# PeixinC/VoiceControlledRobot-VAR

Hardware: AMD Instinct MI355X
Metric: pretext triplets/sec (84x84 RGB + 16 kHz/1 s audio) (higher is better)
Workload: dtype f32; 1 GPU; Kuka+GoogleCommand pretext step, batch 256 per GPU on MI355X, fp32: u8 84x84 image + 2 int16 1 s clips per triplet resident in HBM -> MFCC -> fwd + triplet loss + bwd + Adam (BASELINE.json configs[1]); per_gpu_batch=256, global_batch=256, audio=16 kHz x 1 s int16 x 2, parallelism=dp1, launch=hip-graph replay, head=triplet

## Files before the change

### voicecontrolledrobot-var_amd/csrc/img_tail2.hip

```cpp
#include <stdlib.h>

#include <type_traits>

#include "var_common.h"

namespace {
PH_DECL();
}
#ifdef VAR_PHASES
extern "C" int var_debug_phases_tail2(unsigned long long* out) {
    unsigned long long z[32] = {0};
    if (hipMemcpyFromSymbol(out, HIP_SYMBOL(g_phase), sizeof(z)) != hipSuccess) return -1;
    return hipMemcpyToSymbol(HIP_SYMBOL(g_phase), z, sizeof(z)) == hipSuccess ? 0 : -1;
}
#endif
namespace {
typedef float f32x4t __attribute__((ext_vector_type(4)));

template <bool U8_, int H1_, int RB_, bool TILED_>
struct Tail2Cfg {
    static constexpr bool U8 = U8_, TILED = TILED_;
    static constexpr int CH = 32, H1 = H1_, W1 = H1_, HI = 2 * H1_, HO2 = H1_ / 2;
    static constexpr int RB = RB_, R2 = RB_ / 2, NB = H1_ / RB_;
    static constexpr int A1_ROWS = RB + 1, A1_PITCH = W1, A1_ROW0 = (W1 % 4 == 2) ? 2 : 4;
    static constexpr int A1_PLANE = TILED ? ((A1_ROW0 + A1_ROWS * W1 + 7) / 8) * 8 + 4 : A1_ROW0 + A1_ROWS * W1;
    static constexpr int A1_FLOATS = CH * A1_PLANE;
    static constexpr int G2_ROWS = R2 + 1, G2_PITCH = HO2 + 1;
    static constexpr int G2_PLANE = ((G2_ROWS * G2_PITCH + 15) / 32) * 32 + 16, G2_FLOATS = CH * G2_PLANE;
    static constexpr int G1_PLANE = RB * W1 + ((RB * W1) % 32 == 0 ? 4 : 0), G1_FLOATS = CH * G1_PLANE;
    static constexpr int IM_ROWS = 2 * RB + 1, IM_PITCH = HI + 4, IM_PLANE = IM_ROWS * IM_PITCH, IM_FLOATS = 3 * IM_PLANE;
    static constexpr bool PIPE = !TILED_;
    static constexpr int NBUF = PIPE ? 2 : 1;
    static constexpr int A1S = 0, G2S = A1S + 2 * A1_FLOATS, G1S = G2S + 2 * G2_FLOATS, IMS = G1S + NBUF * G1_FLOATS;
    static constexpr int LUT = IMS + NBUF * IM_FLOATS, ZCELL = LUT + 256;
    static constexpr int LDS_FLOATS = ZCELL + 4;
    static constexpr int LDS_BYTES = LDS_FLOATS * 4;
    static constexpr int NPX2 = R2 * HO2;
    static constexpr int NT2 = (NPX2 + 15) / 16;
    static constexpr int TPW = NT2 % 2 == 0 ? 2 : 1;
    static constexpr int NACC = TPW == 1 ? 2 : 1;
    static constexpr int ND = 2 * NT2 / TPW;
    static constexpr int NT = 64 * (ND + 8);
    static constexpr int KS_W = (NPX2 + 3) / 4;
    static constexpr int NPX1 = RB * W1;
    static constexpr int KS_1 = NPX1 / 4;
    static constexpr int SK = KS_1 <= 48 ? KS_1 / 4 : 8;
    static constexpr int DK = KS_1 <= 48 ? 0 : (((KS_1 - 32 + ND - 1) / ND + 3) / 4) * 4;
    static constexpr int NSL = 4 + (DK ? ND : 0);
    static constexpr int N_A1 = A1_FLOATS / 4;
    static constexpr int P4 = A1_PLANE / 4;
    static constexpr int N_G2 = CH * G2_ROWS * HO2;
    static constexpr int N_IM = 3 * IM_ROWS * (HI / 4);
    static constexpr int L_A1 = TILED ? (N_A1 + 255) / 256 : CH / 4;
    static constexpr int L_G2 = (N_G2 + 255) / 256, L_IM = (N_IM + 255) / 256;
    static constexpr int SLAB0 = 32 * 32 + 32, SLAB1 = 32 * 9 * 32 + 32;
    static_assert(H1 % RB == 0 && RB % 2 == 0 && NPX1 % 4 == 0 && A1_PLANE % 4 == 0 && 4 * SK + DK * ND >= KS_1 && (SK == 8 || SK == 12) && (DK == 0 || DK == 8), "bands, k-step shares");
    static_assert(NT <= 1024 && LDS_BYTES <= 160 * 1024, "one workgroup per CU");
    static_assert(PIPE == (DK == 0), "the pipelined form is the one where role S holds all of conv 1's weight gradient");
    static_assert(NSL * 1024 + NSL * 32 <= 2 * A1_FLOATS, "the end-of-kernel fold scratch aliases the act1 buffers");
    static_assert(CH * HO2 * HO2 < (1 << 15) && CH * G2_PLANE < (1 << 12) && G2_ROWS <= 4, "role S: packed gact2 element table");
    static_assert(3 * HI * HI < (1 << 15) && 3 * IM_PLANE < (1 << 12) && IM_ROWS <= 16, "role S: packed image group table");
};

template <class C>
__global__ void __launch_bounds__(C::NT)
img_tail2_kernel(const float* __restrict__ gy, const float* __restrict__ wd, const float* __restrict__ act1,
                 const void* __restrict__ image, long bstride, const int* __restrict__ bidx,
                 float* __restrict__ slabs0, float* __restrict__ slabs1, int B) {
    extern __shared__ __attribute__((aligned(16))) float lds[];
    using XT = typename std::conditional<C::U8, uint8_t, float>::type;
    const int tid = threadIdx.x, lane = tid & 63, wave = tid >> 6;
    const int q = lane >> 4, l15 = lane & 15;
    const float* lut = lds + C::LUT;
    const int nimg = ((int)blockIdx.x < B) ? (B - 1 - (int)blockIdx.x) / (int)gridDim.x + 1 : 0;
    const int ntl = nimg * C::NB;
    auto tile_img = [&](int j) { return (int)blockIdx.x + (j / C::NB) * (int)gridDim.x; };

    PHR_INIT(3, VAR_PH_THREAD);
    if (tid < 256) lds[C::LUT + tid] = (float)tid / 255.f;
    if (tid < 4) lds[C::ZCELL + tid] = 0.f;
    for (int e = tid; e < 2 * C::G2_FLOATS; e += C::NT) lds[C::G2S + e] = 0.f;
    for (int e = tid; e < C::NBUF * 3 * C::IM_ROWS; e += C::NT) lds[C::IMS + e * C::IM_PITCH + 3] = 0.f;
    __syncthreads();

    float* slab0 = slabs0 + (size_t)blockIdx.x * C::SLAB0;
    float* slab1 = slabs1 + (size_t)blockIdx.x * C::SLAB1;
    f32x4t s_acc[2][2];
    float s_bs[2] = {0.f, 0.f};
#pragma unroll
    for (int a = 0; a < 2; ++a)
#pragma unroll
        for (int b = 0; b < 2; ++b) s_acc[a][b] = {0.f, 0.f, 0.f, 0.f};

    int cbase[2];
#pragma unroll
    for (int kt = 0; kt < 2; ++kt) {
        int col = 16 * kt + l15;
        col = col > 26 ? 26 : col;
        const int tap = col / 3, c = col - tap * 3;
        cbase[kt] = C::IMS + c * C::IM_PLANE + (tap / 3) * C::IM_PITCH + (tap % 3) + 3;
    }
    auto wgrad1_chunk = [&](auto ck, int s_lo, int s_hi, int opq, int g1o = 0, int imo = 0) {
        int m = 4 * s_lo + q + opq;
        int yl = m / C::W1, x = m - yl * C::W1;
        const int ga = C::G1S + g1o + l15 * C::G1_PLANE;
        constexpr int CK = decltype(ck)::value;
        float a0[CK], a1v[CK], b0[CK], b1[CK];
#pragma unroll
        for (int u = 0; u < CK; ++u) {
            const bool live = s_lo + u < s_hi;
            const int pix = 2 * yl * C::IM_PITCH + 2 * x;
            const int ao = live ? ga + m : C::ZCELL, po = live ? pix : 0;
            a0[u] = lds[ao];
            a1v[u] = lds[live ? ao + 16 * C::G1_PLANE : C::ZCELL];
            b0[u] = lds[cbase[0] + imo + po];
            b1[u] = lds[cbase[1] + imo + po];
            m += 4; x += 4;
            if (x >= C::W1) { x -= C::W1; ++yl; }
        }
        __builtin_amdgcn_sched_barrier(0);
#pragma unroll
        for (int u = 0; u < CK; ++u) {
            s_bs[0] += a0[u]; s_bs[1] += a1v[u];
            s_acc[0][0] = __builtin_amdgcn_mfma_f32_16x16x4f32(a0[u], b0[u], s_acc[0][0], 0, 0, 0);
            s_acc[0][1] = __builtin_amdgcn_mfma_f32_16x16x4f32(a0[u], b1[u], s_acc[0][1], 0, 0, 0);
            s_acc[1][0] = __builtin_amdgcn_mfma_f32_16x16x4f32(a1v[u], b0[u], s_acc[1][0], 0, 0, 0);
            s_acc[1][1] = __builtin_amdgcn_mfma_f32_16x16x4f32(a1v[u], b1[u], s_acc[1][1], 0, 0, 0);
        }
        __builtin_amdgcn_sched_barrier(0);
    };

    auto g2_load = [&](auto nl, float* r, int j, int lt) {
        constexpr int NL = decltype(nl)::value, WIN = C::G2_ROWS * C::HO2, CPP = NL / WIN, L = (C::CH + CPP - 1) / CPP;
        const int band = j % C::NB, b = tile_img(j);
        const int cs = lt / WIN, w = lt - cs * WIN, rr = w / C::HO2;
        const int back = (C::R2 * band + rr >= C::HO2) ? C::HO2 : 0;
        const float* pg = gy + (size_t)b * C::CH * C::HO2 * C::HO2 + C::R2 * band * C::HO2 + cs * C::HO2 * C::HO2 + w - back;
#pragma unroll
        for (int i = 0; i < L; ++i) {
            const bool ok = cs < CPP && cs + CPP * i < C::CH;
            r[i] = pg[ok ? CPP * i * C::HO2 * C::HO2 : 0];
        }
    };
    auto g2_store = [&](auto nl, const float* r, int j, int lt) {
        constexpr int NL = decltype(nl)::value, WIN = C::G2_ROWS * C::HO2, CPP = NL / WIN, L = (C::CH + CPP - 1) / CPP;
        const int band = j % C::NB;
        const int cs = lt / WIN, w = lt - cs * WIN, rr = w / C::HO2, ox = w - rr * C::HO2;
        float* dg = lds + C::G2S + (j & 1) * C::G2_FLOATS + cs * C::G2_PLANE + rr * C::G2_PITCH + ox;
        const bool live = C::R2 * band + rr < C::HO2;
#pragma unroll
        for (int i = 0; i < L; ++i)
            if (cs < CPP && cs + CPP * i < C::CH) dg[CPP * i * C::G2_PLANE] = live ? r[i] : 0.f;
    };
    constexpr bool G2_IN_D = C::DK == 0;
    constexpr int NLD_ = 64 * C::ND, L_G2D = (C::CH + NLD_ / (C::G2_ROWS * C::HO2) - 1) / (NLD_ / (C::G2_ROWS * C::HO2));

    auto park_slices = [&](int sl) {
        float* d = lds + sl * 1024;
#pragma unroll
        for (int a = 0; a < 2; ++a)
#pragma unroll
            for (int b = 0; b < 2; ++b)
#pragma unroll
                for (int r = 0; r < 4; ++r) d[(16 * a + 4 * q + r) * 32 + 16 * b + l15] = s_acc[a][b][r];
        float b0 = s_bs[0], b1 = s_bs[1];
        b0 += __shfl_xor(b0, 16, 64); b0 += __shfl_xor(b0, 32, 64);
        b1 += __shfl_xor(b1, 16, 64); b1 += __shfl_xor(b1, 32, 64);
        if (q == 0) { lds[C::NSL * 1024 + sl * 32 + l15] = b0; lds[C::NSL * 1024 + sl * 32 + 16 + l15] = b1; }
    };

    if (wave < C::ND) {
        const int ct = wave & 1, pp = wave >> 1;
        float A[72];
#pragma unroll
        for (int t = 0; t < 72; ++t) A[t] = wd[((t >> 3) * 32 + 4 * (t & 7) + q) * 32 + 16 * ct + l15];
#pragma unroll
        for (int t = 0; t < 72; ++t) asm volatile("" : "+v"(A[t]));
        int mj[C::TPW], mi[C::TPW];
        bool mok[C::TPW];
#pragma unroll
        for (int u = 0; u < C::TPW; ++u) {
            int m = (C::TPW * pp + u) * 16 + l15;
            mok[u] = m < C::NPX2;
            if (!mok[u]) m = 0;
            mj[u] = m / C::HO2; mi[u] = m - mj[u] * C::HO2;
        }
        __syncthreads();
        PHR(0);
        for (int j = 0; j < ntl; ++j) {
            __syncthreads();
            PHR(1);
            float r_g2d[G2_IN_D ? L_G2D : 1];
            int dtid = tid;
            if constexpr (G2_IN_D) {
                asm volatile("" : "+v"(dtid));
                if (j + 1 < ntl) g2_load(std::integral_constant<int, NLD_>{}, r_g2d, j + 1, dtid);
            }
            const int g2 = C::G2S + (j & 1) * C::G2_FLOATS + q * C::G2_PLANE;
            const int a1 = C::A1S + (j & 1) * C::A1_FLOATS;
            constexpr int kCls[9] = {0, 1, 1, 2, 2, 3, 3, 3, 3};
            constexpr int kKy[9] = {1, 1, 1, 0, 2, 0, 0, 2, 2}, kKx[9] = {1, 0, 2, 1, 1, 0, 2, 0, 2};
            int mjb[C::TPW], mib[C::TPW], lb[C::TPW];
#pragma unroll
            for (int u = 0; u < C::TPW; ++u) {
                mjb[u] = mj[u]; mib[u] = mi[u];
                asm volatile("" : "+v"(mjb[u])); asm volatile("" : "+v"(mib[u]));
                lb[u] = g2 + mjb[u] * C::G2_PITCH + mib[u];
            }
            float bb[2][C::TPW][4];
            auto fetch = [&](int buf, int h) {
                const int k = h >> 1, s0 = 4 * (h & 1);
                const int off = (kKy[k] == 0 ? C::G2_PITCH : 0) + (kKx[k] == 0 ? 1 : 0);
#pragma unroll
                for (int ss = 0; ss < 4; ++ss) {
                    bb[buf][0][ss] = lds[lb[0] + off + 4 * (s0 + ss) * C::G2_PLANE];
                    if constexpr (C::TPW == 2) bb[buf][C::TPW - 1][ss] = lds[lb[C::TPW - 1] + off + 4 * (s0 + ss) * C::G2_PLANE];
                }
            };
            f32x4t acc[C::TPW * C::NACC];
#pragma unroll
            for (int u = 0; u < C::TPW * C::NACC; ++u) acc[u] = {0.f, 0.f, 0.f, 0.f};
            fetch(0, 0);
#pragma unroll
            for (int h = 0; h < 18; ++h) {
                const int k = h >> 1;
                if (h + 1 < 18) fetch((h + 1) & 1, h + 1);
                __builtin_amdgcn_sched_barrier(0);
                const int tap = kKy[k] * 3 + kKx[k];
#pragma unroll
                for (int ss = 0; ss < 4; ++ss)
#pragma unroll
                    for (int u = 0; u < C::TPW; ++u)
                        acc[u * C::NACC + ss % C::NACC] = __builtin_amdgcn_mfma_f32_16x16x4f32(A[tap * 8 + 4 * (h & 1) + ss], bb[h & 1][u][ss],
                                                                                    acc[u * C::NACC + ss % C::NACC], 0, 0, 0);
                __builtin_amdgcn_sched_barrier(0);
                if (!(h & 1)) continue;
                if (k + 1 == 9 || kCls[k + 1] != kCls[k]) {
                    const int py = kCls[k] >> 1, px = kCls[k] & 1;
#pragma unroll
                    for (int u = 0; u < C::TPW; ++u) {
                        f32x4t tot = acc[u * C::NACC];
                        if constexpr (C::NACC == 2) tot += acc[u * C::NACC + 1];
                        const int yl = 2 * mjb[u] + py, x = 2 * mib[u] + px;
                        const int mo = a1 + (16 * ct + 4 * q) * C::A1_PLANE + C::A1_ROW0 + (yl + 1) * C::A1_PITCH + x;
                        const int go = C::G1S + (C::PIPE ? (j & 1) * C::G1_FLOATS : 0) + (16 * ct + 4 * q) * C::G1_PLANE + yl * C::W1 + x;
                        float mv[4];
#pragma unroll
                        for (int r = 0; r < 4; ++r) mv[r] = lds[mo + r * C::A1_PLANE];
                        if (mok[u]) {
#pragma unroll
                            for (int r = 0; r < 4; ++r) lds[go + r * C::G1_PLANE] = mv[r] > 0.f ? tot[r] : 0.f;
                        }
#pragma unroll
                        for (int a = 0; a < C::NACC; ++a) acc[u * C::NACC + a] = {0.f, 0.f, 0.f, 0.f};
                    }
                }
            }
            if constexpr (G2_IN_D) {
                asm volatile("" : "+v"(dtid));
                if (j + 1 < ntl) g2_store(std::integral_constant<int, NLD_>{}, r_g2d, j + 1, dtid);
            }
            PHR(2);
            if constexpr (!C::PIPE) __syncthreads();
            PHR(3);
            if constexpr (C::DK == 8) {
                wgrad1_chunk(std::integral_constant<int, 4>{}, 32 + 8 * wave, 32 + 8 * wave + 4, 0);
                wgrad1_chunk(std::integral_constant<int, 4>{}, 32 + 8 * wave + 4, 32 + 8 * wave + 8 < C::KS_1 ? 32 + 8 * wave + 8 : C::KS_1, 0);
            }
            PHR(4);
        }
        PHR_FLUSH();
        if constexpr (C::PIPE) __syncthreads();
        if constexpr (C::DK == 0) __syncthreads();
    } else if (wave < C::ND + 4) {
        const int w = wave - C::ND, nt = w & 1, ctl = w >> 1;
        int aoff[C::KS_W], boff[C::KS_W];
        uint32_t edge = 0;
#pragma unroll
        for (int s = 0; s < C::KS_W; ++s) {
            const int m = 4 * s + q;
            const bool ok = m < C::NPX2;
            const int mm = ok ? m : 0;
            const int r = mm / C::HO2, ox = mm - r * C::HO2;
            aoff[s] = ok ? (16 * nt + l15) * C::G2_PLANE + r * C::G2_PITCH + ox : -1;
            boff[s] = (16 * ctl + l15) * C::A1_PLANE + C::A1_ROW0 + 2 * r * C::A1_PITCH + 2 * ox - 1;
            if (ox == 0) edge |= 1u << s;
        }
        f32x4t acc[9];
#pragma unroll
        for (int t = 0; t < 9; ++t) acc[t] = {0.f, 0.f, 0.f, 0.f};
        float bsum = 0.f;
        __syncthreads();
        PHR(0);
        for (int j = 0; j < ntl; ++j) {
            __syncthreads();
            PHR(1);
            const int g2 = C::G2S + (j & 1) * C::G2_FLOATS, a1 = C::A1S + (j & 1) * C::A1_FLOATS;
            float av[2], bv[2][9];
            auto fetch = [&](int buf, int ss) {
                av[buf] = lds[aoff[ss] < 0 ? C::ZCELL : g2 + aoff[ss]];
#pragma unroll
                for (int t = 0; t < 9; ++t) {
                    const float v = lds[a1 + boff[ss] + (t / 3) * C::A1_PITCH + (t % 3)];
                    bv[buf][t] = (t % 3 == 0 && ((edge >> ss) & 1)) ? 0.f : v;
                }
            };
            fetch(0, 0);
#pragma unroll
            for (int ss = 0; ss < C::KS_W; ++ss) {
                if (ss + 1 < C::KS_W) fetch((ss + 1) & 1, ss + 1);
                __builtin_amdgcn_sched_barrier(0);
                bsum += av[ss & 1];
#pragma unroll
                for (int t = 0; t < 9; ++t) acc[t] = __builtin_amdgcn_mfma_f32_16x16x4f32(av[ss & 1], bv[ss & 1][t], acc[t], 0, 0, 0);
                __builtin_amdgcn_sched_barrier(0);
                if (ss + 1 == C::KS_W / 2) { PHR(2); if constexpr (!C::PIPE) __syncthreads(); PHR(3); }
            }
            PHR(4);
        }
#pragma unroll
        for (int t = 0; t < 9; ++t)
#pragma unroll
            for (int r = 0; r < 4; ++r) slab1[((16 * nt + 4 * q + r) * 9 + t) * 32 + 16 * ctl + l15] = acc[t][r];
        bsum += __shfl_xor(bsum, 16, 64);
        bsum += __shfl_xor(bsum, 32, 64);
        if (ctl == 0 && q == 0) slab1[9216 + 16 * nt + l15] = bsum;
        PHR_FLUSH();
        if constexpr (C::PIPE) __syncthreads();
        if constexpr (C::DK == 0) __syncthreads();
    } else {
        const int sw = wave - C::ND - 4, stid0 = tid - 64 * (C::ND + 4);
        float r_g2[C::L_G2];
        uint32_t r_u8[C::U8 ? C::L_IM : 1];
        float4 r_f4[C::U8 ? 1 : C::L_IM];
        auto make_g2 = [&](int e) -> uint32_t {
            const int ee = e < C::N_G2 ? e : 0;
            const int ch = ee / (C::G2_ROWS * C::HO2), rem = ee - ch * (C::G2_ROWS * C::HO2);
            const int r = rem / C::HO2, ox = rem - r * C::HO2;
            return (uint32_t)(ch * C::HO2 * C::HO2 + r * C::HO2 + ox) | ((uint32_t)(ch * C::G2_PLANE + r * C::G2_PITCH + ox) << 15) |
                   ((uint32_t)r << 27) | (e < C::N_G2 ? 0u : 0x80000000u);
        };
        auto make_im = [&](int e) -> uint32_t {
            const int ee = e < C::N_IM ? e : 0;
            const int c = ee / (C::IM_ROWS * (C::HI / 4)), rem = ee - c * (C::IM_ROWS * (C::HI / 4));
            const int r = rem / (C::HI / 4), g = rem - r * (C::HI / 4);
            return (uint32_t)(c * C::HI * C::HI + r * C::HI + 4 * g) | ((uint32_t)(c * C::IM_PLANE + r * C::IM_PITCH + 4 + 4 * g) << 15) |
                   ((uint32_t)r << 27) | (e < C::N_IM ? 0u : 0x80000000u);
        };
        constexpr bool TAB = C::DK != 0;
        uint32_t t_g2[TAB ? C::L_G2 : 1], t_im[TAB ? C::L_IM : 1];
        if constexpr (TAB) {
#pragma unroll
            for (int i = 0; i < C::L_G2; ++i) t_g2[i] = make_g2(stid0 + 256 * i);
#pragma unroll
            for (int i = 0; i < C::L_IM; ++i) t_im[i] = make_im(stid0 + 256 * i);
        }
        auto e_g2 = [&](int i, int stid) -> uint32_t { if constexpr (TAB) return t_g2[i]; else return make_g2(stid + 256 * i); };
        static_assert(TAB || (C::L_IM == 3 && C::IM_ROWS * (C::HI / 4) <= 256), "image band: a channel per pass");
        auto e_im = [&](int i, int stid) -> uint32_t {
            if constexpr (TAB) return t_im[i];
            else return stid < C::IM_ROWS * (C::HI / 4) ? make_im(stid) : 0x80000000u;
        };
        auto issue_a1g2 = [&](int j, int stid, bool with_g2 = true) {
            const int band = j % C::NB, b = tile_img(j);
            const float* pa = C::TILED ? act1 + (size_t)b * kAct1TiledFloats + (size_t)band * C::A1_FLOATS
                                       : act1 + (size_t)b * C::CH * C::H1 * C::W1;
            float* da = lds + C::A1S + (j & 1) * C::A1_FLOATS;
#pragma unroll
            for (int i = 0; i < C::L_A1; ++i) {
                const int k = sw + 4 * i;
                if constexpr (C::TILED) {
                    if (k * 64 + lane < C::N_A1)
                        __builtin_amdgcn_global_load_lds((const __attribute__((address_space(1))) void*)(pa + k * 256 + 4 * lane),
                                                         (__attribute__((address_space(3))) void*)(da + k * 256), 16, 0, 0);
                } else {
                    static_assert(C::TILED || (C::P4 <= 64 && C::L_A1 * 4 == C::CH), "NCHW gather: a channel per instruction");
                    int off = k * C::H1 * C::W1 + (C::RB * band - 1) * C::W1 - C::A1_ROW0 + 4 * lane;
                    off = off < 0 ? 0 : off;
                    if (lane < C::P4)
                        __builtin_amdgcn_global_load_lds((const __attribute__((address_space(1))) void*)(pa + off),
                                                         (__attribute__((address_space(3))) void*)(da + k * C::A1_PLANE), 16, 0, 0);
                }
            }
            if (!with_g2) return;
            const float* pg = gy + (size_t)b * C::CH * C::HO2 * C::HO2 + C::R2 * band * C::HO2;
#pragma unroll
            for (int i = 0; i < C::L_G2; ++i) {
                const uint32_t tg = e_g2(i, stid);
                const int r = (tg >> 27) & 3;
                const int back = (C::R2 * band + r >= C::HO2) ? C::HO2 : 0;
                r_g2[i] = pg[(int)(tg & 0x7fff) - back];
            }
        };
        auto store_a1g2 = [&](int j, int stid) {
            const int band = j % C::NB;
            float* dg = lds + C::G2S + (j & 1) * C::G2_FLOATS;
#pragma unroll
            for (int i = 0; i < C::L_G2; ++i) {
                const uint32_t tg = e_g2(i, stid);
                const int r = (tg >> 27) & 3;
                if (!(tg >> 31)) dg[(tg >> 15) & 0xfff] = (C::R2 * band + r < C::HO2) ? r_g2[i] : 0.f;
            }
        };
        auto issue_img = [&](int j, int stid) {
            const int band = j % C::NB, b = tile_img(j);
            const int gi = bidx ? bidx[b] : b;
            const int iy0 = 2 * C::RB * band - 1;
            const XT* im = (const XT*)image + (size_t)gi * bstride;
#pragma unroll
            for (int i = 0; i < C::L_IM; ++i) {
                const uint32_t ti = e_im(i, stid);
                const int r = (ti >> 27) & 15;
                const int iy = iy0 + r;
                const int fix = iy < 0 ? C::HI : 0;
                const XT* src = im + (int)(ti & 0x7fff) + iy0 * C::HI + fix;
                if constexpr (!TAB) src = im + (int)(ti & 0x7fff) + i * C::HI * C::HI + iy0 * C::HI + fix;
                if constexpr (C::U8) r_u8[i] = *(const uint32_t*)src;
                else r_f4[i] = *(const float4*)src;
            }
        };
        auto store_img = [&](int j, int stid) {
            const int band = j % C::NB;
            const int iy0 = 2 * C::RB * band - 1;
#pragma unroll
            for (int i = 0; i < C::L_IM; ++i) {
                const uint32_t ti = e_im(i, stid);
                if (ti >> 31) continue;
                const int r = (ti >> 27) & 15;
                const bool rok = iy0 + r >= 0;
                float4 v;
                if constexpr (C::U8) {
                    const uint32_t wv = rok ? r_u8[i] : 0u;
                    v = make_float4(lut[wv & 0xff], lut[(wv >> 8) & 0xff], lut[(wv >> 16) & 0xff], lut[wv >> 24]);
                } else {
                    v = rok ? r_f4[i] : make_float4(0.f, 0.f, 0.f, 0.f);
                }
                *(float4*)(lds + C::IMS + (C::PIPE ? (j & 1) * C::IM_FLOATS : 0) + ((ti >> 15) & 0xfff) + (TAB ? 0 : i * C::IM_PLANE)) = v;
            }
        };
        auto zero_halo = [&](int j, int stid) {
            if constexpr (!C::TILED) {
                if (j % C::NB == 0) {
                    float* da = lds + C::A1S + (j & 1) * C::A1_FLOATS + C::A1_ROW0;
                    for (int e = stid; e < C::CH * (C::W1 / 4); e += 256) {
                        const int ch = e / (C::W1 / 4), o = e - ch * (C::W1 / 4);
                        *(float4*)(da + ch * C::A1_PLANE + 4 * o) = make_float4(0.f, 0.f, 0.f, 0.f);
                    }
                }
            }
        };
        if (ntl > 0) { issue_a1g2(0, stid0); issue_img(0, stid0); store_a1g2(0, stid0); }
        asm volatile("s_waitcnt vmcnt(0)" ::: "memory");
        if (ntl > 0) zero_halo(0, stid0);
        __syncthreads();
        PHR(0);
        for (int j = 0; j < ntl; ++j) {
            __syncthreads();
            PHR(1);
            int stid = stid0;
            asm volatile("" : "+v"(stid));
            store_img(j, stid);
            if constexpr (C::DK != 0) {
                if (j + 1 < ntl) { issue_img(j + 1, stid); issue_a1g2(j + 1, stid); }
                PHR(2);
                __syncthreads();
                PHR(3);
                int z8 = 0;
                asm volatile("" : "+v"(z8));
                wgrad1_chunk(std::integral_constant<int, 8>{}, 8 * sw, 8 * sw + 8, z8);
                PHR(4);
                asm volatile("" : "+v"(stid));
                if (j + 1 < ntl) store_a1g2(j + 1, stid);
                asm volatile("s_waitcnt vmcnt(0)" ::: "memory");
            } else {
                if (j + 1 < ntl) { issue_img(j + 1, stid); issue_a1g2(j + 1, stid, false); }
                PHR(2);
                PHR(3);
                if (j > 0) {
                    int z = 0;
                    asm volatile("" : "+v"(z));
                    const int g1o = ((j - 1) & 1) * C::G1_FLOATS, imo = ((j - 1) & 1) * C::IM_FLOATS;
                    wgrad1_chunk(std::integral_constant<int, 4>{}, C::SK * sw, C::SK * sw + 4, z, g1o, imo);
                    wgrad1_chunk(std::integral_constant<int, 4>{}, C::SK * sw + 4, C::SK * sw + 8, z, g1o, imo);
                    wgrad1_chunk(std::integral_constant<int, 4>{}, C::SK * sw + 8, C::SK * sw + 12, z, g1o, imo);
                }
                PHR(4);
                asm volatile("" : "+v"(stid));
                asm volatile("s_waitcnt vmcnt(0)" ::: "memory");
            }
            if (j + 1 < ntl) zero_halo(j + 1, stid);
            PHR(5);
        }
        PHR_FLUSH();
        if constexpr (C::PIPE) {
            __syncthreads();
            if (ntl > 0) {
                const int g1o = ((ntl - 1) & 1) * C::G1_FLOATS, imo = ((ntl - 1) & 1) * C::IM_FLOATS;
                wgrad1_chunk(std::integral_constant<int, 4>{}, C::SK * sw, C::SK * sw + 4, 0, g1o, imo);
                wgrad1_chunk(std::integral_constant<int, 4>{}, C::SK * sw + 4, C::SK * sw + 8, 0, g1o, imo);
                wgrad1_chunk(std::integral_constant<int, 4>{}, C::SK * sw + 8, C::SK * sw + 12, 0, g1o, imo);
            }
        }
        if constexpr (C::DK == 0) { __syncthreads(); park_slices(sw); }
    }
    if constexpr (C::DK != 0) {
        __syncthreads();
        if (wave < C::ND || wave >= C::ND + 4) park_slices(wave >= C::ND + 4 ? wave - C::ND - 4 : 4 + wave);
    }
    __syncthreads();
    for (int e = tid; e < 1024; e += C::NT) {
        float v = 0.f;
#pragma unroll
        for (int k = 0; k < C::NSL; ++k) v += lds[k * 1024 + e];
        slab0[e] = v;
    }
    if (tid < 32) {
        float v = 0.f;
#pragma unroll
        for (int k = 0; k < C::NSL; ++k) v += lds[C::NSL * 1024 + k * 32 + tid];
        slab0[1024 + tid] = v;
    }
}

template <class C>
int launch_tail2(var_ctx* c, hipStream_t s, int B) {
    ProfScope prof(c, s, TAG_IMG_DGRAD0 + 1);
    static unsigned attr_set = 0;
    if (!(attr_set & var_dev_bit(c))) {
        VAR_HIP_CHECK(c, hipFuncSetAttribute((const void*)img_tail2_kernel<C>, hipFuncAttributeMaxDynamicSharedMemorySize,
                                             C::LDS_BYTES));
        attr_set |= var_dev_bit(c);
    }
    const int G = B < kTail2G ? B : kTail2G;
    c->wg_groups[0] = G;
    c->wg_groups[1] = G;
    hipLaunchKernelGGL(img_tail2_kernel<C>, dim3(G), dim3(C::NT), C::LDS_BYTES, s, c->gact[2], c->wpack + c->kl.img_d[1],
                       c->act[1], c->saved_image, c->saved_bstride, c->saved_index, c->slabs + img_slab_offset(0),
                       c->slabs + img_slab_offset(1), B);
    VAR_HIP_CHECK(c, hipGetLastError());
    return VAR_OK;
}
}

int launch_img_bwd_tail2(var_ctx* c, hipStream_t s, int B) {
    if (c->fwd_plan.act1_tiled != (c->H == 84)) {
        VAR_SET_ERR(c, "image backward: the saved forward left act1 in the other layout");
        return VAR_ERR_STATE;
    }
    if (c->H == 96) return c->saved_u8 ? launch_tail2<Tail2Cfg<true, 48, 4, false>>(c, s, B) : launch_tail2<Tail2Cfg<false, 48, 4, false>>(c, s, B);
    return c->saved_u8 ? launch_tail2<Tail2Cfg<true, 42, 6, true>>(c, s, B) : launch_tail2<Tail2Cfg<false, 42, 6, true>>(c, s, B);
}
```

Measured before the change: 919,800 triplets/s.

## Overlap tail2 prologue loads with LDS init and vectorize epilogue slab writes

```diff
diff --git a/voicecontrolledrobot-var_amd/csrc/img_tail2.hip b/voicecontrolledrobot-var_amd/csrc/img_tail2.hip
--- a/voicecontrolledrobot-var_amd/csrc/img_tail2.hip
+++ b/voicecontrolledrobot-var_amd/csrc/img_tail2.hip
@@ -56,8 +56,11 @@
     static constexpr int SLAB0 = 32 * 32 + 32, SLAB1 = 32 * 9 * 32 + 32;
     static_assert(H1 % RB == 0 && RB % 2 == 0 && NPX1 % 4 == 0 && A1_PLANE % 4 == 0 && 4 * SK + DK * ND >= KS_1 && (SK == 8 || SK == 12) && (DK == 0 || DK == 8), "bands, k-step shares");
     static_assert(NT <= 1024 && LDS_BYTES <= 160 * 1024, "one workgroup per CU");
+    static_assert(G2S % 4 == 0 && G2_FLOATS % 2 == 0, "the gact2 buffers are zeroed 16 bytes at a time");
     static_assert(PIPE == (DK == 0), "the pipelined form is the one where role S holds all of conv 1's weight gradient");
-    static_assert(NSL * 1024 + NSL * 32 <= 2 * A1_FLOATS, "the end-of-kernel fold scratch aliases the act1 buffers");
+    static constexpr int W_PARK = NSL * 1024 + NSL * 32;
+    static_assert(W_PARK % 4 == 0 && SLAB0 % 4 == 0 && SLAB1 % 4 == 0 && W_PARK + SLAB1 <= 2 * A1_FLOATS,
+                  "the end-of-kernel fold scratch and role W's parked slab alias the act1 buffers");
     static_assert(CH * HO2 * HO2 < (1 << 15) && CH * G2_PLANE < (1 << 12) && G2_ROWS <= 4, "role S: packed gact2 element table");
     static_assert(3 * HI * HI < (1 << 15) && 3 * IM_PLANE < (1 << 12) && IM_ROWS <= 16, "role S: packed image group table");
 };
@@ -77,11 +80,17 @@
     auto tile_img = [&](int j) { return (int)blockIdx.x + (j / C::NB) * (int)gridDim.x; };
 
     PHR_INIT(3, VAR_PH_THREAD);
-    if (tid < 256) lds[C::LUT + tid] = (float)tid / 255.f;
-    if (tid < 4) lds[C::ZCELL + tid] = 0.f;
-    for (int e = tid; e < 2 * C::G2_FLOATS; e += C::NT) lds[C::G2S + e] = 0.f;
-    for (int e = tid; e < C::NBUF * 3 * C::IM_ROWS; e += C::NT) lds[C::IMS + e * C::IM_PITCH + 3] = 0.f;
-    __syncthreads();
+    auto fills_and_barrier = [&]() {
+        constexpr int NF = 64 * (C::ND + 4);
+        if (tid < 256) lds[C::LUT + tid] = (float)tid / 255.f;
+        if (tid < 4) lds[C::ZCELL + tid] = 0.f;
+        if (tid < NF) {
+            for (int e = tid; e < 2 * C::G2_FLOATS / 4; e += NF) *(float4*)(lds + C::G2S + 4 * e) = make_float4(0.f, 0.f, 0.f, 0.f);
+            for (int e = tid; e < C::NBUF * 3 * C::IM_ROWS; e += NF) lds[C::IMS + e * C::IM_PITCH + 3] = 0.f;
+        }
+        asm volatile("s_waitcnt lgkmcnt(0)\n\ts_barrier" ::: "memory");
+        PHR(6);
+    };
 
     float* slab0 = slabs0 + (size_t)blockIdx.x * C::SLAB0;
     float* slab1 = slabs1 + (size_t)blockIdx.x * C::SLAB1;
@@ -136,10 +145,9 @@
         const int cs = lt / WIN, w = lt - cs * WIN, rr = w / C::HO2;
         const int back = (C::R2 * band + rr >= C::HO2) ? C::HO2 : 0;
         const float* pg = gy + (size_t)b * C::CH * C::HO2 * C::HO2 + C::R2 * band * C::HO2 + cs * C::HO2 * C::HO2 + w - back;
-#pragma unroll
-        for (int i = 0; i < L; ++i) {
-            const bool ok = cs < CPP && cs + CPP * i < C::CH;
-            r[i] = pg[ok ? CPP * i * C::HO2 * C::HO2 : 0];
+        if (cs < CPP) {
+#pragma unroll
+            for (int i = 0; i < L; ++i) r[i] = pg[cs + CPP * i < C::CH ? CPP * i * C::HO2 * C::HO2 : 0];
         }
     };
     auto g2_store = [&](auto nl, const float* r, int j, int lt) {
@@ -154,8 +162,9 @@
     };
     constexpr bool G2_IN_D = C::DK == 0;
     constexpr int NLD_ = 64 * C::ND, L_G2D = (C::CH + NLD_ / (C::G2_ROWS * C::HO2) - 1) / (NLD_ / (C::G2_ROWS * C::HO2));
-
-    auto park_slices = [&](int sl) {
+    constexpr int NL0 = G2_IN_D ? NLD_ : 256, L_G20 = (C::CH + NL0 / (C::G2_ROWS * C::HO2) - 1) / (NL0 / (C::G2_ROWS * C::HO2));
+
+    auto park_slices = [&](int sl, int q, int l15) {
         float* d = lds + sl * 1024;
 #pragma unroll
         for (int a = 0; a < 2; ++a)
@@ -169,11 +178,15 @@
         if (q == 0) { lds[C::NSL * 1024 + sl * 32 + l15] = b0; lds[C::NSL * 1024 + sl * 32 + 16 + l15] = b1; }
     };
 
-    if (wave < C::ND) {
+    if (tid < 64 * C::ND) {
         const int ct = wave & 1, pp = wave >> 1;
+        float r_g20[G2_IN_D ? L_G20 : 1];
+        if constexpr (G2_IN_D) { if (ntl > 0) g2_load(std::integral_constant<int, NL0>{}, r_g20, 0, tid); }
         float A[72];
 #pragma unroll
         for (int t = 0; t < 72; ++t) A[t] = wd[((t >> 3) * 32 + 4 * (t & 7) + q) * 32 + 16 * ct + l15];
+        fills_and_barrier();
+        if constexpr (G2_IN_D) { if (ntl > 0) g2_store(std::integral_constant<int, NL0>{}, r_g20, 0, tid); }
 #pragma unroll
         for (int t = 0; t < 72; ++t) asm volatile("" : "+v"(A[t]));
         int mj[C::TPW], mi[C::TPW];
@@ -269,11 +282,13 @@
             }
             PHR(4);
         }
-        PHR_FLUSH();
         if constexpr (C::PIPE) __syncthreads();
         if constexpr (C::DK == 0) __syncthreads();
-    } else if (wave < C::ND + 4) {
+    } else if (tid < 64 * (C::ND + 4)) {
         const int w = wave - C::ND, nt = w & 1, ctl = w >> 1;
+        float r_g20[G2_IN_D ? 1 : L_G20];
+        if constexpr (!G2_IN_D) { if (ntl > 0) g2_load(std::integral_constant<int, NL0>{}, r_g20, 0, tid - 64 * C::ND); }
+        fills_and_barrier();
         int aoff[C::KS_W], boff[C::KS_W];
         uint32_t edge = 0;
 #pragma unroll
@@ -290,6 +305,7 @@
 #pragma unroll
         for (int t = 0; t < 9; ++t) acc[t] = {0.f, 0.f, 0.f, 0.f};
         float bsum = 0.f;
+        if constexpr (!G2_IN_D) { if (ntl > 0) g2_store(std::integral_constant<int, NL0>{}, r_g20, 0, tid - 64 * C::ND); }
         __syncthreads();
         PHR(0);
         for (int j = 0; j < ntl; ++j) {
@@ -318,15 +334,16 @@
             }
             PHR(4);
         }
-#pragma unroll
-        for (int t = 0; t < 9; ++t)
-#pragma unroll
-            for (int r = 0; r < 4; ++r) slab1[((16 * nt + 4 * q + r) * 9 + t) * 32 + 16 * ctl + l15] = acc[t][r];
         bsum += __shfl_xor(bsum, 16, 64);
         bsum += __shfl_xor(bsum, 32, 64);
-        if (ctl == 0 && q == 0) slab1[9216 + 16 * nt + l15] = bsum;
-        PHR_FLUSH();
-        if constexpr (C::PIPE) __syncthreads();
+        PHR(10);
+        __syncthreads();
+        float* pw = lds + C::W_PARK;
+#pragma unroll
+        for (int t = 0; t < 9; ++t)
+#pragma unroll
+            for (int r = 0; r < 4; ++r) pw[((16 * nt + 4 * q + r) * 9 + t) * 32 + 16 * ctl + l15] = acc[t][r];
+        if (ctl == 0 && q == 0) pw[9216 + 16 * nt + l15] = bsum;
         if constexpr (C::DK == 0) __syncthreads();
     } else {
         const int sw = wave - C::ND - 4, stid0 = tid - 64 * (C::ND + 4);
@@ -350,8 +367,6 @@
         constexpr bool TAB = C::DK != 0;
         uint32_t t_g2[TAB ? C::L_G2 : 1], t_im[TAB ? C::L_IM : 1];
         if constexpr (TAB) {
-#pragma unroll
-            for (int i = 0; i < C::L_G2; ++i) t_g2[i] = make_g2(stid0 + 256 * i);
 #pragma unroll
             for (int i = 0; i < C::L_IM; ++i) t_im[i] = make_im(stid0 + 256 * i);
         }
@@ -449,9 +464,17 @@
                 }
             }
         };
-        if (ntl > 0) { issue_a1g2(0, stid0); issue_img(0, stid0); store_a1g2(0, stid0); }
+        if (ntl > 0) { issue_a1g2(0, stid0, false); issue_img(0, stid0); }
+        PHR(7);
+        fills_and_barrier();
+        if constexpr (TAB) {
+#pragma unroll
+            for (int i = 0; i < C::L_G2; ++i) t_g2[i] = make_g2(stid0 + 256 * i);
+        }
+        PHR(8);
         asm volatile("s_waitcnt vmcnt(0)" ::: "memory");
         if (ntl > 0) zero_halo(0, stid0);
+        PHR(9);
         __syncthreads();
         PHR(0);
         for (int j = 0; j < ntl; ++j) {
@@ -491,7 +514,6 @@
             if (j + 1 < ntl) zero_halo(j + 1, stid);
             PHR(5);
         }
-        PHR_FLUSH();
         if constexpr (C::PIPE) {
             __syncthreads();
             if (ntl > 0) {
@@ -501,25 +523,34 @@
                 wgrad1_chunk(std::integral_constant<int, 4>{}, C::SK * sw + 8, C::SK * sw + 12, 0, g1o, imo);
             }
         }
-        if constexpr (C::DK == 0) { __syncthreads(); park_slices(sw); }
+        PHR(10);
+        if constexpr (C::DK == 0) { __syncthreads(); park_slices(sw, q, l15); }
     }
     if constexpr (C::DK != 0) {
-        __syncthreads();
-        if (wave < C::ND || wave >= C::ND + 4) park_slices(wave >= C::ND + 4 ? wave - C::ND - 4 : 4 + wave);
+        if (tid < 64 * C::ND || tid >= 64 * (C::ND + 4)) {
+            __syncthreads();
+            int te = tid;
+            asm volatile("" : "+v"(te));
+            const int we = te >> 6;
+            park_slices(we >= C::ND + 4 ? we - C::ND - 4 : 4 + we, (te & 63) >> 4, te & 15);
+        }
     }
     __syncthreads();
-    for (int e = tid; e < 1024; e += C::NT) {
-        float v = 0.f;
-#pragma unroll
-        for (int k = 0; k < C::NSL; ++k) v += lds[k * 1024 + e];
-        slab0[e] = v;
+    PHR(11);
+    for (int e = tid; e < C::SLAB1 / 4; e += C::NT) ((float4*)slab1)[e] = ((const float4*)(lds + C::W_PARK))[e];
+    for (int e = tid; e < C::SLAB0 / 4; e += C::NT) {
+        const float* src = lds + (e < 256 ? 4 * e : C::NSL * 1024 + 4 * (e - 256));
+        const int pitch = e < 256 ? 1024 : 32;
+        float4 v = make_float4(0.f, 0.f, 0.f, 0.f);
+#pragma unroll
+        for (int k = 0; k < C::NSL; ++k) {
+            const float4 x = *(const float4*)(src + k * pitch);
+            v.x += x.x; v.y += x.y; v.z += x.z; v.w += x.w;
+        }
+        ((float4*)slab0)[e] = v;
     }
-    if (tid < 32) {
-        float v = 0.f;
-#pragma unroll
-        for (int k = 0; k < C::NSL; ++k) v += lds[C::NSL * 1024 + k * 32 + tid];
-        slab0[1024 + tid] = v;
-    }
+    PHR(12);
+    PHR_FLUSH();
 }
 
 template <class C>
```

After: 921,500 triplets/s (median of 6 runs). No clear change (+0.2%).
